# maca/crdt-graph

Measured on AMD Instinct MI355X. Metric: merged ops/sec (whole node) on 10M-op batch, higher is better.
Workload: dtype int64; 1 GPU; flat10m: 10000000 ops per GPU, one document per GPU; replicas=64, window=256, guard=0, parallelism=documents sharded by id over 1 GPU(s)

## Files before the change

crdt-graph_amd/csrc/merge.hip:

```cpp

#include <cstring>

#include "engine.h"
#include "listrank.h"
#include "scan.h"

namespace crdtm {


struct Work {
  uint8_t* st;
  uint32_t* cur;
  uint32_t* leaf;
  uint32_t* addpar;
  uint32_t* dtime;
  uint8_t* dead;
  uint32_t* maxadd;
  uint4* nrec;
  uint32_t* tag;
};

__device__ __forceinline__ uint32_t op_len(const OpsDev& o, uint32_t i) { return o.off[i + 1] - o.off[i]; }

struct Quad {
  uint32_t cnt;
  uint8_t kind[4];
  long long ts[4];
  uint32_t off[5];
};

__device__ __forceinline__ void load_quad(const OpsDev& o, uint32_t i0, Quad& q) {
  if (i0 + 4 <= o.n) {
    q.cnt = 4;
    const uchar4 k = *reinterpret_cast<const uchar4*>(o.kind + i0);
    q.kind[0] = k.x;
    q.kind[1] = k.y;
    q.kind[2] = k.z;
    q.kind[3] = k.w;
    const longlong2 a = *reinterpret_cast<const longlong2*>(o.ts + i0);
    const longlong2 b = *reinterpret_cast<const longlong2*>(o.ts + i0 + 2);
    q.ts[0] = a.x;
    q.ts[1] = a.y;
    q.ts[2] = b.x;
    q.ts[3] = b.y;
    const uint4 f = *reinterpret_cast<const uint4*>(o.off + i0);
    q.off[0] = f.x;
    q.off[1] = f.y;
    q.off[2] = f.z;
    q.off[3] = f.w;
    q.off[4] = o.off[i0 + 4];
  } else {
    q.cnt = o.n - i0;
#pragma unroll
    for (uint32_t k = 0; k < 4; ++k) {
      const bool v = k < q.cnt;
      q.kind[k] = v ? o.kind[i0 + k] : 0;
      q.ts[k] = v ? o.ts[i0 + k] : 0;
    }
#pragma unroll
    for (uint32_t k = 0; k < 5; ++k) q.off[k] = k <= q.cnt ? o.off[i0 + k] : 0;
  }
}

__device__ __forceinline__ void store_quad_u8(uint8_t* p, uint32_t i0, uint32_t cnt, const uint8_t v[4]) {
  if (cnt == 4) {
    *reinterpret_cast<uchar4*>(p + i0) = make_uchar4(v[0], v[1], v[2], v[3]);
  } else {
    for (uint32_t k = 0; k < cnt; ++k) p[i0 + k] = v[k];
  }
}

#define QUAD_LOOP(i0, n)                                                                           \
  for (uint32_t i0 = 4 * (blockIdx.x * blockDim.x + threadIdx.x); i0 < (n); i0 += 4 * gridDim.x * blockDim.x)

#define QUAD_LOOP_XCD(i0, n)                                                                       \
  const uint32_t nq_ = ((n) + 3) / 4;                                                              \
  const bool x8_ = (gridDim.x & 7) == 0;                                                           \
  const uint32_t xc_ = x8_ ? blockIdx.x & 7 : 0, xy_ = x8_ ? blockIdx.x >> 3 : blockIdx.x;         \
  const uint32_t cq_ = (x8_ ? gridDim.x >> 3 : gridDim.x) * blockDim.x, xs_ = x8_ ? 8 : 1;         \
  for (uint32_t j_ = xc_, qd_ = xc_ * cq_ + xy_ * blockDim.x + threadIdx.x, i0 = 4 * qd_;         \
       j_ * cq_ < nq_; j_ += xs_, qd_ = j_ * cq_ + xy_ * blockDim.x + threadIdx.x, i0 = 4 * qd_)   \
    if (qd_ < nq_)

static uint32_t env_grid(const char* name, uint32_t def) {
  const char* e = getenv(name);
  const int g = e ? atoi(e) : 0;
  return g >= 8 && g <= (1 << 20) ? static_cast<uint32_t>(g) : def;
}

inline uint32_t quad_grid(uint64_t n) {
  const uint64_t g = (((n + 3) / 4) + BLOCK - 1) / BLOCK;
  if (g >= 2048) return 2048;
  return g < 8 ? static_cast<uint32_t>(g ? g : 1) : static_cast<uint32_t>((g + 7) & ~7ULL);
}



constexpr uint32_t REP_DIRECT = 4096;
constexpr uint32_t PRE_T = 1024;
template <uint32_t PB>
__global__ void __launch_bounds__(PB) __attribute__((amdgpu_waves_per_eu(PB == 1024 ? 8 : 4, 8))) k_pre(OpsDev o, uint2* rng, DevResult* dres) {
  __shared__ __attribute__((aligned(16))) uint32_t rlo[REP_DIRECT];
  __shared__ __attribute__((aligned(16))) uint32_t rhi[REP_DIRECT];
  for (uint32_t j = threadIdx.x; j < REP_DIRECT / 4; j += blockDim.x) {
    reinterpret_cast<uint4*>(rlo)[j] = make_uint4(NONE, NONE, NONE, NONE);
    reinterpret_cast<uint4*>(rhi)[j] = make_uint4(0u, 0u, 0u, 0u);
  }
  __syncthreads();
  uint32_t mx = 0, bad = 0, neg = 0, ndel = 0, maxr = 0;
  auto fold = [&](const Quad& q) {
#pragma unroll
    for (uint32_t k = 0; k < 4; ++k) {
      if (k >= q.cnt) break;
      const uint32_t L = q.off[k + 1] - q.off[k];
      mx = max(mx, L);
      if (q.kind[k] != CRDTM_ADD) {
        ++ndel;
        continue;
      }
      const long long ts = q.ts[k];
      if (ts >= TWO53 || ts <= -TWO53) {
        bad = 1;
      } else if (ts < 0) {
        neg = 1;
      } else if (L >= 1 && ts != 0) {
        const uint32_t r = static_cast<uint32_t>(static_cast<uint64_t>(ts) >> 32), c = static_cast<uint32_t>(ts);
        maxr = max(maxr, r);
        if (r < REP_DIRECT) {
          if (c < rlo[r]) atomicMin(&rlo[r], c);
          if (c > rhi[r]) atomicMax(&rhi[r], c);
        } else {
          atomicMin(&rng[r].x, c);
          atomicMax(&rng[r].y, c);
        }
      }
    }
  };
  {
    const uint32_t qs = 4 * gridDim.x * blockDim.x;
    uint32_t i0 = 4 * (blockIdx.x * blockDim.x + threadIdx.x);
    for (; i0 + qs < o.n; i0 += 2 * qs) {
      Quad qa, qb;
      load_quad(o, i0, qa);
      load_quad(o, i0 + qs, qb);
      fold(qa);
      fold(qb);
    }
    if (i0 < o.n) {
      Quad qa;
      load_quad(o, i0, qa);
      fold(qa);
    }
  }
  auto mxf = [](uint32_t a, uint32_t b) { return a > b ? a : b; };
  maxr = block_reduce_t<PB>(maxr, 0u, mxf);
  for (uint32_t j = threadIdx.x; j <= maxr && j < REP_DIRECT; j += blockDim.x) {
    if (rlo[j] <= rhi[j]) {
      atomicMin(&rng[j].x, rlo[j]);
      atomicMax(&rng[j].y, rhi[j]);
    }
  }
  mx = block_reduce_t<PB>(mx, 0u, mxf);
  bad = block_reduce_t<PB>(bad, 0u, mxf);
  neg = block_reduce_t<PB>(neg, 0u, mxf);
  ndel = block_reduce_t<PB>(ndel, 0u, [](uint32_t a, uint32_t b) { return a + b; });
  if (threadIdx.x == 0) {
    if (mx) atomicMax(&dres->max_len, mx);
    if (bad) atomicOr(&dres->bad_range, 1u);
    if (neg) atomicOr(&dres->has_negative, 1u);
    if (ndel) atomicAdd(&dres->n_del, ndel);
    if (maxr) atomicMax(&dres->max_replica, maxr);
  }
}

__global__ void __launch_bounds__(BLOCK) k_path_range(OpsDev o, DevResult* dres) {
  const uint64_t np = o.n_path, npair = np / 2;
  auto out = [](long long v) { return v >= TWO53 || v <= -TWO53; };
  uint32_t bad = 0;
  const uint64_t ps = static_cast<uint64_t>(gridDim.x) * blockDim.x;
  uint64_t p = blockIdx.x * static_cast<uint64_t>(blockDim.x) + threadIdx.x;
  for (; p + 3 * ps < npair; p += 4 * ps) {
    longlong2 v[4];
#pragma unroll
    for (uint32_t u = 0; u < 4; ++u) v[u] = *reinterpret_cast<const longlong2*>(o.path + 2 * (p + u * ps));
#pragma unroll
    for (uint32_t u = 0; u < 4; ++u)
      if (out(v[u].x) || out(v[u].y)) bad = 1;
  }
  for (; p < npair; p += ps) {
    const longlong2 v = *reinterpret_cast<const longlong2*>(o.path + 2 * p);
    if (out(v.x) || out(v.y)) bad = 1;
  }
  if ((np & 1) && blockIdx.x == 0 && threadIdx.x == 0 && out(o.path[np - 1])) bad = 1;
  bad = block_max(bad);
  if (threadIdx.x == 0 && bad) atomicOr(&dres->bad_range, 1u);
}

constexpr uint32_t REP_SPEC = 256;
template <uint32_t PB, bool BLIND>
__global__ void __launch_bounds__(PB) k_pre_ts(const long long* __restrict__ ts, const uint8_t* __restrict__ kind,
                                               const uint32_t* __restrict__ off, uint32_t n, uint2* rng,
                                               uint32_t* base, DevResult* dres) {
  __shared__ uint32_t rlo[REP_SPEC], rhi[REP_SPEC];
  __shared__ uint32_t s_last;
  __shared__ unsigned long long sw[PB / 64];
  for (uint32_t j = threadIdx.x; j < REP_SPEC; j += PB) {
    rlo[j] = NONE;
    rhi[j] = 0;
  }
  __syncthreads();
  uint32_t bad = 0, neg = 0, maxr = 0, vfail = 0;
  auto fold = [&](long long t) {
    if (t >= TWO53 || t <= -TWO53) {
      bad = 1;
    } else if (t < 0) {
      neg = 1;
    } else if (t != 0) {
      const uint32_t r = static_cast<uint32_t>(static_cast<uint64_t>(t) >> 32), c = static_cast<uint32_t>(t);
      maxr = max(maxr, r);
      if (r < REP_SPEC) {
        if (BLIND || c < rlo[r]) atomicMin(&rlo[r], c);
        if (BLIND || c > rhi[r]) atomicMax(&rhi[r], c);
      }
    }
  };
  {
    const longlong2* t2 = reinterpret_cast<const longlong2*>(ts);
    const uchar2* k2 = reinterpret_cast<const uchar2*>(kind);
    const uint2* o2 = reinterpret_cast<const uint2*>(off);
    auto verify = [&](uint32_t p, uchar2 k, uint2 f) {
      vfail |= (k.x | k.y) != CRDTM_ADD || f.x != 2 * p || f.y != 2 * p + 1;
    };
    const uint32_t np = n / 2, gs = gridDim.x * PB;
    uint32_t p = blockIdx.x * PB + threadIdx.x;
    for (; p + 3 * gs < np; p += 4 * gs) {
      longlong2 v[4];
      uchar2 k[4];
      uint2 f[4];
#pragma unroll
      for (uint32_t u = 0; u < 4; ++u) {
        v[u] = t2[p + u * gs];
        k[u] = k2[p + u * gs];
        f[u] = o2[p + u * gs];
      }
#pragma unroll
      for (uint32_t u = 0; u < 4; ++u) {
        fold(v[u].x);
        fold(v[u].y);
        verify(p + u * gs, k[u], f[u]);
      }
    }
    for (; p < np; p += gs) {
      const longlong2 v = t2[p];
      fold(v.x);
      fold(v.y);
      verify(p, k2[p], o2[p]);
    }
    if (blockIdx.x == 0 && threadIdx.x == 0) {
      if (n & 1) {
        fold(ts[n - 1]);
        vfail |= kind[n - 1] != CRDTM_ADD || off[n - 1] != n - 1;
      }
      vfail |= off[n] != n;
    }
  }
  auto mxf = [](uint32_t a, uint32_t b) { return a > b ? a : b; };
  maxr = block_reduce_t<PB>(maxr, 0u, mxf);
  for (uint32_t j = threadIdx.x; j <= maxr && j < REP_SPEC; j += PB)
    if (rlo[j] <= rhi[j]) {
      atomicMin(&rng[j].x, rlo[j]);
      atomicMax(&rng[j].y, rhi[j]);
    }
  bad = block_reduce_t<PB>(bad, 0u, mxf);
  neg = block_reduce_t<PB>(neg, 0u, mxf);
  vfail = block_reduce_t<PB>(vfail, 0u, mxf);
  if (threadIdx.x == 0) {
    if (vfail) atomicOr(&dres->spec_fail, 1u);
    if (bad) atomicOr(&dres->bad_range, 1u);
    if (neg) atomicOr(&dres->has_negative, 1u);
    if (maxr) atomicMax(&dres->max_replica, maxr);
    s_last = __hip_atomic_fetch_add(&dres->pre_done, 1u, __ATOMIC_ACQ_REL, __HIP_MEMORY_SCOPE_AGENT) ==
             gridDim.x - 1;
  }
  __syncthreads();
  if (!s_last) return;
  const uint32_t nr =
      min(__hip_atomic_load(&dres->max_replica, __ATOMIC_ACQUIRE, __HIP_MEMORY_SCOPE_AGENT), REP_SPEC - 1) + 1;
  const uint32_t lane = threadIdx.x & 63, wave = threadIdx.x / 64;
  unsigned long long sz = 0;
  if (threadIdx.x < nr) {
    const uint32_t lo = __hip_atomic_load(&rng[threadIdx.x].x, __ATOMIC_RELAXED, __HIP_MEMORY_SCOPE_AGENT);
    const uint32_t hi = __hip_atomic_load(&rng[threadIdx.x].y, __ATOMIC_RELAXED, __HIP_MEMORY_SCOPE_AGENT);
    sz = lo <= hi ? static_cast<unsigned long long>(hi - lo) + 1ULL : 0ULL;
  }
  const unsigned long long inc = wave_incl_scan64(sz);
  if (lane == 63) sw[wave] = inc;
  __syncthreads();
  unsigned long long pre = inc - sz, tot = 0;
  for (uint32_t w = 0; w < PB / 64; ++w) {
    if (w < wave) pre += sw[w];
    tot += sw[w];
  }
  if (threadIdx.x < nr) base[threadIdx.x] = static_cast<uint32_t>(pre < NONE ? pre : NONE);
  if (threadIdx.x == 0) {
    const uint32_t q = static_cast<uint32_t>(tot < NONE - 64 ? tot : NONE - 64);
    dres->range_total = q;
    dres->fl_nw = (q + 63) / 64;
  }
}

__global__ void __launch_bounds__(BLOCK) k_work_init(OpsDev o, Work w) {
  GRID_STRIDE(i, o.n) {
    w.st[i] = op_len(o, i) == 0 ? ST_INVALID : ST_PENDING;
    w.cur[i] = o.n;
    w.addpar[i] = NONE;
    w.dtime[i] = NONE;
    w.tag[i] = NONE;
  }
}

__global__ void __launch_bounds__(BLOCK) k_nrec_init(OpsDev o, Work w) {
  GRID_STRIDE(i, o.n) {
    const uint32_t b = o.off[i], L = o.off[i + 1] - b;
    w.nrec[i] = make_uint4(b, L | (static_cast<uint32_t>(ST_PENDING) << 16), NONE, NONE);
  }
}
__device__ __forceinline__ uint32_t nrec_len(const uint4& r) { return r.y & 0xFFFFu; }
__device__ __forceinline__ uint32_t nrec_st(const uint4& r) { return (r.y >> 16) & 0xFFu; }
__device__ __forceinline__ bool nrec_dead(const uint4& r) { return (r.y >> 24) & 1u; }

__global__ void __launch_bounds__(BLOCK) k_range_base(const uint2* rng, uint32_t* base, DevResult* dres) {
  __shared__ unsigned long long sw[BLOCK / 64];
  const uint32_t nr = dres->max_replica + 1;
  const int lane = threadIdx.x & 63, wave = threadIdx.x >> 6;
  unsigned long long carry = 0;
  for (uint32_t r0 = 0; r0 < nr; r0 += BLOCK) {
    const uint32_t r = r0 + threadIdx.x;
    unsigned long long sz = 0;
    if (r < nr) {
      const uint2 g = rng[r];
      sz = g.x <= g.y ? static_cast<unsigned long long>(g.y - g.x) + 1ULL : 0ULL;
    }
    const unsigned long long inc = wave_incl_scan64(sz);
    if (lane == 63) sw[wave] = inc;
    __syncthreads();
    unsigned long long pre = carry + (inc - sz), tot = 0;
    for (int w = 0; w < BLOCK / 64; ++w) {
      if (w < wave) pre += sw[w];
      tot += sw[w];
    }
    if (r < nr) base[r] = static_cast<uint32_t>(pre < NONE ? pre : NONE);
    carry += tot;
    __syncthreads();
  }
  if (threadIdx.x == 0) dres->range_total = static_cast<uint32_t>(carry < NONE ? carry : NONE);
}

__global__ void __launch_bounds__(BLOCK) k_range_reset(uint2* rng, uint32_t nr, const DevResult* dres) {
  if (nr == 0) nr = dres->max_replica + 1;
  GRID_STRIDE(r, nr) rng[r] = make_uint2(NONE, 0u);
}

void range_reset(crdtm_ctx* c, uint32_t nr) {
// ... 2144 lines not shown
struct RunSizeGen {
  static constexpr bool kStriped = true;
  static constexpr bool kEpilogue = false;
  const uint32_t* tk;
  const uint32_t* offk;
  __device__ __forceinline__ bool aligned(uint64_t b) const {
    return ((reinterpret_cast<uintptr_t>(tk + b) | reinterpret_cast<uintptr_t>(offk + b)) & 15) == 0;
  }
  __device__ __forceinline__ uint4 load4(uint64_t b) const {
    const uint4 t = *reinterpret_cast<const uint4*>(tk + b), f = *reinterpret_cast<const uint4*>(offk + b);
    return make_uint4(t.x | (f.x & SEGF), t.y | (f.y & SEGF), t.z | (f.z & SEGF), t.w | (f.w & SEGF));
  }
  __device__ __forceinline__ void load(uint64_t b, uint64_t n, uint32_t* v) const {
#pragma unroll
    for (int j = 0; j < DS_ITEMS; ++j) v[j] = b + j < n ? (tk[b + j] | (offk[b + j] & SEGF)) : 0u;
  }
};

__global__ void __launch_bounds__(BLOCK) k_run_w2(RunArr a, uint32_t Q, const uint32_t* sarr, const uint32_t* pk,
                                                  const uint32_t* xs, const uint32_t* offk) {
  if (a.qd) Q = min(*a.qd, Q);
  RUN_LOOP(k) {
    const uint32_t f = offk[k], r = sarr[k], p = pk[k];
    if (p > Q) continue;
    const uint32_t ex = (f & SEGF) ? 0u : (xs[k - 1] & ~SEGF);
    a.rr[r].y = ex + (f & ~SEGF);
  }
}

__device__ __forceinline__ uint32_t run_S(const uint32_t* xs, uint32_t k) { return k ? xs[k - 1] : 0u; }

__global__ void __launch_bounds__(BLOCK) k_run_gstart(RunArr a, uint32_t Q, const uint32_t* pk, RunMask rm,
                                                      uint32_t* groot) {
  if (a.qd) Q = min(*a.qd, Q);
  const uint32_t R = *a.nR;
  const uint32_t lane = threadIdx.x & 63;
  for (uint32_t k0 = blockIdx.x * blockDim.x; k0 < R; k0 += gridDim.x * blockDim.x) {
    const uint32_t k = k0 + threadIdx.x;
    const uint32_t p = k < R ? pk[k] : Q + 1;
    const uint32_t P = p < Q ? run_of(rm, p) : NONE;
    uint32_t Pp = __shfl_up(P, 1, 64), Pn = __shfl_down(P, 1, 64);
    if (k >= R) continue;
    if (p == Q && (k == 0 || pk[k - 1] != Q)) *groot = k;
    if (p >= Q) continue;
    if (lane == 0) Pp = k ? (pk[k - 1] < Q ? run_of(rm, pk[k - 1]) : NONE) : NONE;
    if (lane == 63 || k + 1 == R) Pn = k + 1 < R && pk[k + 1] < Q ? run_of(rm, pk[k + 1]) : NONE;
    if (Pp != P) a.rr[P].z = k;
    if (Pn != P) a.rr[P].w = k + 1;
  }
}

__global__ void __launch_bounds__(BLOCK) k_run_w(RunArr a, uint32_t Q, const uint32_t* sarr, const uint32_t* pk,
                                                 const uint32_t* xs, const uint32_t* groot, RunMask rm) {
  if (a.qd) Q = min(*a.qd, Q);
  RUN_LOOP(k) {
    const uint32_t r = sarr[k], p = pk[k];
    if (p > Q) continue;
    if (p == Q) {
      a.rr[r].y = run_S(xs, k) - run_S(xs, *groot);
    } else {
      const uint32_t P = run_of(rm, p);
      a.rr[r].y = run_S(xs, k) - run_S(xs, a.rr[P].z) + (p - a.hh[P].x) + 1u;
    }
  }
}

__global__ void __launch_bounds__(BLOCK) k_run_pos(RunArr a, DevResult* dres) {
  RUN_LOOP(r) {
    const uint4 e = a.rr[r];
    uint32_t s = e.y, d = 0;
    for (uint32_t x = e.x; x != NONE;) {
      if (++d > RUN_MAXD) {
        atomicOr(&dres->run_fail, 1u);
        break;
      }
      const uint4 f = a.rr[x];
      s += f.y;
      x = f.x;
    }
    a.posh[r] = s;
  }
}

__global__ void __launch_bounds__(BLOCK) k_run_expand(RunArr a, uint32_t Q, uint32_t K, RunMask rm,
                                                      const uint32_t* pk, const uint32_t* xs, const uint32_t* qc,
                                                      uint32_t* doc, FlatRec fr, uint32_t lds_iters, uint32_t seg) {
  extern __shared__ uint32_t smw[];
  Q = fr.q(Q);
  const uint32_t iters = (Q + gridDim.x * blockDim.x - 1) / (gridDim.x * blockDim.x);
  const bool mlds = iters <= lds_iters;
  const uint32_t wpb = blockDim.x >> 6;
  if (mlds) {
    const uint32_t nw = (Q + 63) >> 6;
    for (uint32_t j = threadIdx.x; j < iters * wpb; j += blockDim.x) {
      const uint32_t w = (blockIdx.x + (j / wpb) * gridDim.x) * wpb + j % wpb;
      const unsigned long long m = w < nw ? rm.hm[w] : 0ULL;
      smw[3 * j] = static_cast<uint32_t>(m);
      smw[3 * j + 1] = static_cast<uint32_t>(m >> 32);
      smw[3 * j + 2] = w < nw ? rm.hb[w] : 0u;
    }
  }
  __syncthreads();
  const uint32_t lane = threadIdx.x & 63, stride = gridDim.x * blockDim.x;
  const unsigned long long below = (2ULL << lane) - 1ULL;
  auto run_at = [&](uint32_t it, uint32_t q) -> uint32_t {
    unsigned long long mq;
    uint32_t bq;
    if (mlds) {
      const uint32_t* e = smw + 3 * (it * wpb + (threadIdx.x >> 6));
      mq = (static_cast<unsigned long long>(e[1]) << 32) | e[0];
      bq = e[2];
    } else {
      mq = rm.hm[q >> 6];
      bq = rm.hb[q >> 6];
    }
    return bq + static_cast<uint32_t>(__popcll(mq & below)) - 1u;
  };
  uint32_t q0 = blockIdx.x * blockDim.x;
  uint2 hn = make_uint2(0u, ABSENT);
  uint32_t pn = 0;
  uint4 en = make_uint4(0u, 0u, 0u, 0u);
  auto fetch = [&](uint32_t it, uint32_t q) {
    if (q < Q) {
      const uint32_t r = run_at(it, q);
      hn = a.hh[r];
      pn = a.posh[r];
      en = a.rr[r];
    }
  };
  fetch(0, q0 + threadIdx.x);
  for (uint32_t it = 0; q0 < Q; q0 += stride, ++it) {
    const uint32_t q = q0 + threadIdx.x;
    const uint2 h = hn;
    const uint32_t ph = pn;
    const uint4 er = en;
    hn = make_uint2(0u, ABSENT);
    if (q0 + stride < Q) fetch(it + 1, q + stride);
    if (q >= Q || h.y == ABSENT) continue;
    uint32_t p = ph + (q - h.x);
    const uint32_t e0 = er.z, e1 = er.w;
    if (e1 > e0) {
      uint32_t lo = e0, hi = e1;
      while (lo < hi) {
        const uint32_t mid = (lo + hi) >> 1;
        if (pk[mid] < q) lo = mid + 1;
        else hi = mid;
      }
      if (lo > e0) p += seg ? (xs[lo - 1] & ~SEGF) : xs[lo - 1] - run_S(xs, e0);
    }
    if (p < K) doc[p] = 1 + (qc ? qc[q] : q);
  }
}

__global__ void __launch_bounds__(BLOCK) k_fl_count(uint32_t Q, const uint32_t* ep, uint32_t* cnt) {
  uint32_t hot = 0;
  GRID_STRIDE(x, Q) {
    const uint32_t d = ep[x];
    if (d == ABSENT) continue;
    if (d == Q) ++hot;
    else atomicAdd(&cnt[d], 1u);
  }
  hot = block_sum(hot);
  if (threadIdx.x == 0 && hot) atomicAdd(&cnt[Q], hot);
}

thread_local crdtm_ctx* g_prof = nullptr;

void mark_begin(crdtm_ctx* c, hipStream_t st) {
  if (!c->profile) return;
  if (c->pending) hipEventDestroy(c->pending);
  c->pending = nullptr;
  hipEvent_t e;
  if (hipEventCreate(&e) != hipSuccess) return;
  hipEventRecord(e, st);
  c->pending = e;
}

void mark(crdtm_ctx* c, const char* name, hipStream_t st) {
  if (!c->profile || !c->pending) return;
  hipEvent_t e;
  if (hipEventCreate(&e) != hipSuccess) return;
  hipEventRecord(e, st);
  c->marks.push_back({name, c->pending, e});
  c->pending = nullptr;
}

template <class T>
static int grow_array(T*& p, uint64_t old_n, uint64_t new_n) {
  T* q = nullptr;
  HIP_CHECK(hipMalloc(&q, new_n * sizeof(T) + 256));
  if (p) {
    if (old_n) HIP_CHECK(hipMemcpy(q, p, old_n * sizeof(T), hipMemcpyDeviceToDevice));
    HIP_CHECK(hipFree(p));
  }
  p = q;
  return CRDTM_OK;
}

DevStore::~DevStore() {
  void* ps[] = {d.s_key, d.s_next, d.s_src, d.s_child, d.s_dict, d.s_flags, d.d_sent,
                d.d_owner, d.l_kind, d.l_ts, d.l_val, d.l_off, d.l_path, d.doc};
  for (void* p : ps)
    if (p) hipFree(p);
}

static int grow_tree_arrays(crdtm_tree* t, const TreeCaps& need);

int grow_tree(crdtm_tree* t, const TreeCaps& need) {
  if (!t->store) t->store = std::make_shared<DevStore>();
  const int r = grow_tree_arrays(t, need);
  t->store->d = t->d;
  return r;
}

static int grow_tree_arrays(crdtm_tree* t, const TreeCaps& need) {
  HIP_CHECK(hipStreamSynchronize(t->ctx->stream));
  TreeCaps& c = t->cap;
  auto bump = [](uint64_t have, uint64_t want) { return want <= have ? have : (want + want / 4 + 1024); };
  if (need.slots > c.slots) {
    uint64_t n = bump(c.slots, need.slots);
    int r = 0;
    if ((r = grow_array(t->d.s_key, t->n_slots, n)) || (r = grow_array(t->d.s_next, t->n_slots, n)) ||
        (r = grow_array(t->d.s_src, t->n_slots, n)) || (r = grow_array(t->d.s_child, t->n_slots, n)) ||
        (r = grow_array(t->d.s_dict, t->n_slots, n)) || (r = grow_array(t->d.s_flags, t->n_slots, n)))
      return r;
    c.slots = n;
  }
  if (need.dicts > c.dicts) {
    uint64_t n = bump(c.dicts, need.dicts);
    int r = 0;
    if ((r = grow_array(t->d.d_sent, t->n_dicts, n)) || (r = grow_array(t->d.d_owner, t->n_dicts, n))) return r;
    c.dicts = n;
  }
// ... 310 lines not shown
      if ((r = scan_excl_u32(logidx, logidx, n, &dr->log_n, ws, s))) return r;
      if ((r = scan_excl_u32(plen, plen, n, &dr->log_npath, ws, s))) return r;
      LAUNCH(k_log, dim3(g), dim3(BLOCK), 0, s, o, st, t->d, 0u, 0u, logidx, plen);
      LAUNCH(k_log_tail, dim3(1), dim3(1), 0, s, t->d, 0u, &dr->log_n, 0u, &dr->log_npath);
    }
    uint32_t* qc = nullptr;
    if (!fr.qd && Q != K) {
      qc = fb.qc = ws.alloc<uint32_t>(Q);
      LAUNCH(k_fl_present, dim3(gq), dim3(BLOCK), 0, s, Q, fr, qc);
      if ((r = scan_excl_u32(qc, qc, Q, nullptr, ws, s))) return r;
    }
    static const uint32_t mask_u = [] {
      const char* e = getenv("CRDTM_MASK_U");
      const uint32_t u = e ? static_cast<uint32_t>(atoi(e)) : RM_MASK_UNROLL;
      return (u == 1 || u == 4) ? u : RM_MASK_UNROLL;
    }();
    static const uint32_t mask_grid = env_grid("CRDTM_MASK_GRID", 1024);
    const uint32_t gw = std::max<uint32_t>(1, std::min<uint32_t>(mask_grid, (NW + mask_u * (BLOCK / 64) - 1) /
                                                                                 (mask_u * (BLOCK / 64))));
    const size_t mshm = maxr + 1 <= HOST_RANGES ? 3 * (maxr + 1) * sizeof(uint32_t) : 0;
    const bool dq = fr.qd != nullptr;
    auto mask_launch = [&](auto kern, const char* name) {
      prof_begin(s);
      hipLaunchKernelGGL(kern, dim3(gw), dim3(BLOCK), mshm, s, fr, Q, hm, hc, t->d, qc, logidx, o, ix, maxr + 1,
                         check ? dr : nullptr, c->rtab);
      prof_mark(name, s);
    };
    static const bool diag_mask2 = [] {
      const char* e = getenv("CRDTM_DIAG_MASK2");
      return e && e[0] == '1';
    }();
    if (diag_mask2) mask_launch(dq ? k_run_mask<RM_MASK_UNROLL, true> : k_run_mask<RM_MASK_UNROLL, false>, "k_run_mask");
    if (mask_u == 1) mask_launch(dq ? k_run_mask<1, true> : k_run_mask<1, false>, "k_run_mask");
    else if (mask_u == 4) mask_launch(dq ? k_run_mask<4, true> : k_run_mask<4, false>, "k_run_mask");
    else mask_launch(dq ? k_run_mask<RM_MASK_UNROLL, true> : k_run_mask<RM_MASK_UNROLL, false>, "k_run_mask");
    if ((r = dscan<SumOp, false>(ArrGen{hc}, hb, NW, &dr->run_count, ws, s, nullptr, fr.qd ? &dr->fl_nw : nullptr,
                                 "k_dscan_runs")))
      return r;
    static const bool run_v2 = [] {
      const char* e = getenv("CRDTM_RUN_V2");
      return !(e && e[0] == '0');
    }();
    ra.hasch = run_v2 ? ws.alloc<uint8_t>(Q + 1) : nullptr;
    static const uint32_t heads_grid = env_grid("CRDTM_HEADS_GRID", 4096);
    LAUNCH(k_run_heads, dim3(grid_for(64ULL * NW, BLOCK, heads_grid)), dim3(BLOCK), 0, s, fr, Q, fb.rm, ra.hh,
           ra.hasch);
    ra.rr = ws.alloc<uint4>(Q + 1);
    ra.ca = ws.alloc<unsigned long long>(Q + 1);
    uint32_t* kinv = ws.alloc<uint32_t>(Q + 1);
    ra.kinv = kinv;
    ra.posh = ws.alloc<uint32_t>(Q + 1);
    uint32_t* sk[2] = {ws.alloc<uint32_t>(Q + 1), ws.alloc<uint32_t>(Q + 1)};
    uint32_t* sv[2] = {ws.alloc<uint32_t>(Q + 1), ws.alloc<uint32_t>(Q + 1)};
    uint32_t* xs = ws.alloc<uint32_t>(Q + 1);
    uint32_t* groot = fb.cnt;
    static const uint32_t run_grid = env_grid("CRDTM_RUN_GRID", 2048);
    const uint32_t gr = grid_for(Q, BLOCK, run_grid);
    static const bool ep_coh = [] {
      const char* e = getenv("CRDTM_EP_COHERENT");
      return e && e[0] == '1';
    }();
    if (ep_coh) LAUNCH(k_run_ep<true>, dim3(gr), dim3(BLOCK), 0, s, ra, Q, fb.rm, fr, sk[0], sv[0]);
    else LAUNCH(k_run_ep<false>, dim3(gr), dim3(BLOCK), 0, s, ra, Q, fb.rm, fr, sk[0], sv[0]);
    uint32_t *pk = nullptr, *sarr = nullptr;
    {
      uint32_t sbits = 8;
      while (sbits < 32 && ((static_cast<uint64_t>(Q) + 1) >> sbits) != 0) sbits += 8;
      if ((r = radix_sort_pairs(sk[0], sv[0], sk[1], sv[1], ra.nR, Q, sbits, ws, s, &pk, &sarr, kinv))) return r;
      ra.tk = pk == sk[0] ? sk[1] : sk[0];
      if (!run_v2) LAUNCH(k_run_gstart, dim3(gr), dim3(BLOCK), 0, s, ra, Q, pk, fb.rm, groot);
    }
    if (run_v2) {
      uint32_t* offk = ws.alloc<uint32_t>(Q + 1);
      LAUNCH(k_run_sizes, dim3(gr), dim3(BLOCK), 0, s, ra, Q, sarr, pk, fb.rm, offk);
      if ((r = dscan<SegSumOp, true>(RunSizeGen{ra.tk, offk}, xs, Q, nullptr, ws, s, nullptr, ra.nR, "k_dscan_seg")))
        return r;
      LAUNCH(k_run_w2, dim3(gr), dim3(BLOCK), 0, s, ra, Q, sarr, pk, xs, offk);
    } else {
      LAUNCH(k_run_tree_up, dim3(gr), dim3(BLOCK), 0, s, ra, sarr);
      if ((r = dscan<SumOp, true>(ArrGen{ra.tk}, xs, Q, nullptr, ws, s, nullptr, ra.nR, "k_dscan_xs"))) return r;
      LAUNCH(k_run_w, dim3(gr), dim3(BLOCK), 0, s, ra, Q, sarr, pk, xs, groot, fb.rm);
    }
    LAUNCH(k_run_pos, dim3(gr), dim3(BLOCK), 0, s, ra, dr);
    static const uint32_t ex_grid = env_grid("CRDTM_EX_GRID", 2048);
    const uint32_t gx = grid_for(Q, BLOCK, ex_grid);
    const uint32_t ex_iters = (Q + gx * BLOCK - 1) / (gx * BLOCK);
    LAUNCH(k_run_expand, dim3(gx), dim3(BLOCK),
           ex_iters <= EX_ITERS ? 3 * ex_iters * (BLOCK / 64) * sizeof(uint32_t) : 0, s, ra, Q, K, fb.rm, pk, xs, qc,
           t->d.doc, fr, ex_iters <= EX_ITERS ? ex_iters : 0u, run_v2 ? 1u : 0u);
    static const uint32_t next_grid = env_grid("CRDTM_NEXT_GRID", 1u << 20);
    fb.rep = ws.alloc<long long>(2 * static_cast<uint64_t>(maxr) + 2);
    RepCollect rc{o, 0u, c->rtab, fb.rep, &dr->n_replica_out, dr->rep_inline, check ? c->crange : nullptr};
    const bool rep_here = !(all_applied && !log_done);
    if (rep_here) rc.nr = maxr + 1;
    LAUNCH(k_fl_next, dim3(grid_for(K, BLOCK, next_grid)), dim3(BLOCK), 0, s, K, t->d.doc, t->d, t->cap.slots, rc);
    if (rep_here) return CRDTM_OK;
    if (all_applied && !log_done) fl_log_copy(c, o, t->d, simple);
  } else if (all_applied && !log_done) {
    fl_log_copy(c, o, t->d, simple);
  }
  if (!fb.rep) fb.rep = ws.alloc<long long>(2 * static_cast<uint64_t>(maxr) + 2);
  LAUNCH(k_fl_rep_collect, dim3(grid_for(maxr + 1)), dim3(BLOCK), 0, s, o, maxr + 1, c->rtab, fb.rep,
         &dr->n_replica_out, dr->rep_inline, check ? c->crange : nullptr);
  return CRDTM_OK;
}

static int flat_order_fallback(crdtm_tree* t, uint32_t Q, uint32_t K, FlatBufs& fb) {
  crdtm_ctx* c = t->ctx;
  hipStream_t s = c->stream;
  Arena& ws = c->ws;
  DevResult* dr = c->dres;
  const uint32_t U = Q + 1;
  const uint32_t gq = grid_for(Q);
  uint32_t* anc = fb.anc;
  uint32_t* cnt = fb.cnt;
  uint32_t* fill = fb.fill;
  uint32_t* qc = fb.qc;
  int r;
  {
    RunArr ra{};
    ra.hh = fb.hh;
    LAUNCH(k_run_ep_slots, dim3(gq), dim3(BLOCK), 0, s, ra, Q, fb.rm, fb.fr, anc);
  }
  uint32_t* carr = ws.alloc<uint32_t>(U);
  uint32_t* ns = ws.alloc<uint32_t>(U);
  HIP_CHECK(hipMemsetAsync(cnt, 0, (U + 1) * sizeof(uint32_t), s));
  HIP_CHECK(hipMemsetAsync(fill, 0, (U + 1) * sizeof(uint32_t), s));
  LAUNCH(k_fl_count, dim3(grid_for(Q, BLOCK, 2048)), dim3(BLOCK), 0, s, Q, anc, cnt);
  uint32_t* n_child = &dr->n_sentinels;
  if ((r = scan_excl_u32(cnt, cnt, U + 1, n_child, ws, s))) return r;
  LAUNCH(k_fl_scatter, dim3(gq), dim3(BLOCK), 0, s, Q, anc, cnt, fill, carr);
  {
    const uint32_t gb = grid_for(Q, BLOCK, 2048);
    uint32_t* bc = ws.alloc<uint32_t>(gb + 1);
    LAUNCH(k_fl_root_count, dim3(gb), dim3(BLOCK), 0, s, Q, anc, bc);
    if ((r = scan_excl_u32(bc, bc, gb, nullptr, ws, s))) return r;
    LAUNCH(k_fl_root_place, dim3(gb), dim3(BLOCK), 0, s, Q, anc, bc, cnt, carr);
  }
  if ((r = segmented_sort_desc_id(cnt, U, carr, U, ws, s, dr, Q))) return r;
  LAUNCH(k_fl_links, dim3(gq), dim3(BLOCK), 0, s, anc, cnt, n_child, carr, ns);
  if ((r = list_rank_fused(FlatEulerSrc{Q, anc, cnt, carr, ns}, 2ULL * U, 2 * Q, FlatDocSink{Q, t->d.doc, qc},
                           ws, s)))
    return r;
  LAUNCH(k_fl_next, dim3(grid_for(K)), dim3(BLOCK), 0, s, K, t->d.doc, t->d, t->cap.slots, RepCollect{});
  return CRDTM_OK;
}

static int apply_flat(crdtm_tree* t, const OpsDev& o, const TsIndex& ix, uint32_t Q, uint32_t maxr, uint8_t* st,
                      uint8_t* st_out, crdtm_result* res, bool simple, RangeReset& rr, bool devq = false,
                      bool* done = nullptr) {
  if (done) *done = true;
  crdtm_ctx* c = t->ctx;
  hipStream_t s = c->stream;
  Arena& ws = c->ws;
  DevResult* dr = c->dres;
  const uint32_t n = o.n;
  const uint32_t g = grid_for(n);
  const uint32_t U = Q + 1;
  FlatBufs fb{};
  fb.anc = ws.alloc<uint32_t>(U);
  fb.cnt = ws.alloc<uint32_t>(U + 1);
  fb.fill = ws.alloc<uint32_t>(U + 1);
  int r;
  auto grow_for = [&](uint32_t K, uint32_t applied) -> int {
    TreeCaps need = t->cap;
    need.slots = std::max<uint64_t>(need.slots, 1ULL + K + 1);
    need.dicts = std::max<uint64_t>(need.dicts, 2);
    need.log = std::max<uint64_t>(need.log, t->log_n + applied + 1);
    need.lpath = std::max<uint64_t>(need.lpath, t->log_npath + o.n_path + 1);
    need.doc = std::max<uint64_t>(need.doc, 1ULL + K);
    if (need.slots > t->cap.slots || need.dicts > t->cap.dicts || need.log > t->cap.log ||
        need.lpath > t->cap.lpath || need.doc > t->cap.doc)
      return grow_tree(t, need);
// ... 75 lines not shown
    LAUNCH(k_reset_root, dim3(1), dim3(1), 0, s, t->d.s_next, nullptr);
    launch_pre(c, o, s);
    LAUNCH(k_range_base, dim3(1), dim3(BLOCK), 0, s, c->crange, const_cast<uint32_t*>(ix.base), dr);
    rr.armed = true;
  }
  LAUNCH(k_fl_rep_collect, dim3(grid_for(maxr + 1)), dim3(BLOCK), 0, s, o, maxr + 1, c->rtab, nullptr, nullptr,
         nullptr, nullptr);
  LAUNCH(k_fl_stat_reset, dim3(1), dim3(1), 0, s, dr);
  LAUNCH(k_fl_status, dim3(quad_grid(n)), dim3(BLOCK), 0, s, o, st, ix, Q, fb.fr, t->timestamp, c->rtab, dr);
  if ((r = sync_read(c))) return r;
  if (c->hres->dup_fix) {
    LAUNCH(k_fl_rep_collect, dim3(grid_for(maxr + 1)), dim3(BLOCK), 0, s, o, maxr + 1, c->rtab, nullptr, nullptr,
           nullptr, nullptr);
    LAUNCH(k_fl_stat_reset, dim3(1), dim3(1), 0, s, dr);
    LAUNCH(k_fl_status, dim3(quad_grid(n)), dim3(BLOCK), 0, s, o, st, ix, Q, fb.fr, t->timestamp, c->rtab, dr);
    if ((r = sync_read(c))) return r;
  }
  const DevResult h1 = *c->hres;
  if (h1.bad_range) return CRDTM_E_RANGE;
  uint32_t guard = 0;
  const long long new_ts = t->timestamp + h1.own_ok_adds - t->own_bias;
  if (replica_of(new_ts) != replica_of(t->timestamp)) guard |= G_REPLICA_DRIFT;
  res->guard = guard;
  if (guard || h1.err_index != NONE)
    LAUNCH(k_fl_rep_collect, dim3(grid_for(maxr + 1)), dim3(BLOCK), 0, s, o, maxr + 1, c->rtab, nullptr, nullptr,
           nullptr, nullptr);
  if (guard) {
    r = run_replay(t, o, st, res, guard);
    if (r == CRDTM_OK && st_out)
      LAUNCH(k_status_out, dim3(g), dim3(BLOCK), 0, s, st, n,
             res->err_index >= 0 ? static_cast<uint32_t>(res->err_index) : NONE, st_out);
    return r;
  }
  res->path_taken = CRDTM_PATH_CLOSED_FORM;
  if (h1.err_index != NONE) {
    uint8_t est = 0;
    HIP_CHECK(hipMemcpy(&est, st + h1.err_index, 1, hipMemcpyDeviceToHost));
    res->code = est == ST_INVALID ? CRDTM_INVALID_PATH : CRDTM_OPERATION_FAILED;
    res->err_index = h1.err_index;
    if (st_out) LAUNCH(k_status_out, dim3(g), dim3(BLOCK), 0, s, st, n, h1.err_index, st_out);
    return CRDTM_OK;
  }
  const uint32_t K = h1.n_adds_applied;
  const bool all_applied = h1.n_applied == n;
  if ((r = grow_for(K, h1.n_applied))) return r;
  LAUNCH(k_fl_commit_reset, dim3(1), dim3(1), 0, s, dr);
  if ((r = flat_order_commit(t, o, ix, Q, maxr, st, K, all_applied, spec, simple, false, fb))) return r;
  if (st_out) LAUNCH(k_status_out, dim3(g), dim3(BLOCK), 0, s, st, n, NONE, st_out);
  if ((r = sync_read(c))) return r;
  if (c->hres->run_fail && (r = flat_order_fallback(t, Q, K, fb))) return r;
  return finish(K, h1.n_applied, h1.n_already, all_applied ? o.n_path : c->hres->log_npath, new_ts);
}

static int apply_core(crdtm_tree* t, const OpsDev& o, uint8_t* st_out, crdtm_result* res) {
  crdtm_ctx* c = t->ctx;
  hipStream_t s = c->stream;
  Arena& ws = c->ws;
  const uint32_t n = o.n;
  res->err_index = -1;
  res->code = CRDTM_OK;
  if (n == 0) {
    res->path_taken = CRDTM_PATH_CLOSED_FORM;
    t->last_begin = t->last_end = t->log_n;
    return CRDTM_OK;
  }
  Work w;
  w.st = ws.alloc<uint8_t>(n);
  uint32_t* rbase = ws.alloc<uint32_t>(RID_SLOTS + 1);
  DevResult* dr = c->dres;
  const bool dres_ready = c->dres_ready;
  c->dres_ready = false;
  const char* fe = getenv("CRDTM_FORCE_REPLAY");
  const bool force_replay = fe && fe[0] == '1';
  static const bool spec_on = [] {
    const char* e = getenv("CRDTM_FLAT_SPEC");
    return !(e && e[0] == '0');
  }();
  if (spec_on && !force_replay && t->n_slots == 1 && t->log_n == 0 && !t->remerge && o.n_path == n) {
    uint32_t b = 8;
    while (b < 32 && ((static_cast<uint64_t>(n) + 2) >> b) != 0) b += 8;
    const uint64_t qcap = std::min<uint64_t>(std::max<uint64_t>((1ULL << b) - 2, 65536), 4ULL * n + 65536);
    if (qcap + 2 < (1ULL << FR_ABITS) - 1) {
      if (!dres_ready) LAUNCH(k_dres_init, dim3(1), dim3(64), 0, s, dr);
      static const uint32_t pre_grid = env_grid("CRDTM_PRE_GRID", 256);
      static const bool pre_blind = [] {
        const char* e = getenv("CRDTM_PRE_BLIND");
        return e && e[0] == '1';
      }();
      const uint32_t gp = static_cast<uint32_t>(std::min<uint64_t>((n / 2 + PRE_T - 1) / PRE_T + 1, pre_grid));
      if (pre_blind)
        LAUNCH((k_pre_ts<PRE_T, true>), dim3(gp), dim3(PRE_T), 0, s, o.ts, o.kind, o.off, n, c->crange, rbase, dr);
      else
        LAUNCH((k_pre_ts<PRE_T, false>), dim3(gp), dim3(PRE_T), 0, s, o.ts, o.kind, o.off, n, c->crange, rbase, dr);
      RangeReset spec_clean{c};
      TsIndex ix;
      ix.rng = c->crange;
      ix.base = rbase;
      ix.dense = 1;
      ix.h = TsHash{nullptr, nullptr, 0};
      ix.first = nullptr;
      bool done = false;
      int rs = apply_flat(t, o, ix, static_cast<uint32_t>(qcap), REP_SPEC - 1, w.st, st_out, res, true, spec_clean,
                          true, &done);
      if (rs || done) return rs;
    }
  }
  LAUNCH(k_dres_init, dim3(1), dim3(64), 0, s, dr);
  launch_pre(c, o, s);
  LAUNCH(k_range_base, dim3(1), dim3(BLOCK), 0, s, c->crange, rbase, dr);
  RangeReset keep_clean{c};
  int r;
  if ((r = sync_read(c))) return r;
  keep_clean.nr = c->hres->max_replica + 1;
  if (c->hres->bad_range) return CRDTM_E_RANGE;
  const uint32_t maxlen = c->hres->max_len;
  if (t->max_depth < maxlen) t->max_depth = maxlen;
  const uint32_t g = grid_for(n);
  if (force_replay || t->n_slots != 1 || t->log_n != 0) {
    if (o.n_path) {
      LAUNCH(k_path_range, dim3(std::min<uint32_t>(grid_for(o.n_path / 2 + 1), 1024)), dim3(BLOCK), 0, s, o, dr);
      if ((r = sync_read(c))) return r;
      if (c->hres->bad_range) return CRDTM_E_RANGE;
    }
    r = run_replay(t, o, w.st, res, force_replay ? G_FORCED : G_NOT_FRESH);
    if (r == CRDTM_OK && st_out)
      LAUNCH(k_status_out, dim3(g), dim3(BLOCK), 0, s, w.st, n,
             res->err_index >= 0 ? static_cast<uint32_t>(res->err_index) : NONE, st_out);
    return r;
  }
  const uint32_t maxr = c->hres->max_replica;
  const uint64_t range_total = c->hres->range_total;
  TsIndex ix;
  ix.rng = c->crange;
  ix.base = rbase;
  ix.dense = (!c->hres->has_negative && range_total <= 4ULL * n + 65536) ? 1u : 0u;
  const bool flat = maxlen == 1 && c->hres->n_del == 0;
  const bool levels = !flat && maxlen <= MAXLV_BUCKET;
  const bool side_range = !(ix.dense && flat) && !levels && o.n_path;
  if (side_range) {
    HIP_CHECK(hipEventRecord(c->ev_fork, s));
    HIP_CHECK(hipStreamWaitEvent(c->side, c->ev_fork, 0));
    LAUNCH(k_path_range, dim3(std::min<uint32_t>(grid_for(o.n_path / 2 + 1), 1024)), dim3(BLOCK), 0, c->side, o,
           dr);
    HIP_CHECK(hipEventRecord(c->ev_join, c->side));
  }
  auto range_ok = [&]() -> int {
    return c->hres->bad_range ? CRDTM_E_RANGE : CRDTM_OK;
  };
  if (ix.dense) {
    ix.h = TsHash{nullptr, nullptr, 0};
    ix.first = nullptr;
    if (flat)
      return apply_flat(t, o, ix, static_cast<uint32_t>(range_total), maxr, w.st, st_out, res, o.n_path == n,
                        keep_clean);
    ix.first = ws.alloc<uint32_t>(range_total + 1);
    HIP_CHECK(hipMemsetAsync(ix.first, 0xFF, (range_total + 1) * sizeof(uint32_t), s));
    const uint32_t nrep = maxr + 1 <= HOST_RANGES ? maxr + 1 : 0u;
    LAUNCH(k_index_store, dim3(quad_grid(n)), dim3(BLOCK), 3 * nrep * sizeof(uint32_t), s, o, ix, nrep);
    LAUNCH(k_index_fix, dim3(quad_grid(n)), dim3(BLOCK), 3 * nrep * sizeof(uint32_t), s, o, ix, nrep);
  } else {
    const uint32_t H = pow2_at_least(2 * static_cast<uint64_t>(n));
    ix.first = nullptr;
    ix.h.keys = ws.alloc<unsigned long long>(H);
    ix.h.vals = ws.alloc<uint32_t>(H);
    ix.h.mask = H - 1;
    HIP_CHECK(hipMemsetAsync(ix.h.keys, 0, H * sizeof(unsigned long long), s));
    HIP_CHECK(hipMemsetAsync(ix.h.vals, 0xFF, H * sizeof(uint32_t), s));
// ... 585 lines not shown
```

Before: 16.67 billion ops/s.

## Software-pipeline pre-pass loads, batch run_expand searches, skip redundant global atomics

The timestamp pre-pass now double-buffers groups of four loads so the next group is in flight while the current one is folded, with a masked tail loop. The run_expand kernel is templated on the LDS mode and processes two queries per thread, interleaving their binary searches so memory loads overlap. Global atomicMin, atomicMax and max_replica updates are skipped when a relaxed load shows they would not change the value. Grid env lookups are re-read under test hooks, and the extra live registers may reduce occupancy.

```diff
diff --git a/crdt-graph_amd/csrc/merge.hip b/crdt-graph_amd/csrc/merge.hip
--- a/crdt-graph_amd/csrc/merge.hip
+++ b/crdt-graph_amd/csrc/merge.hip
@@ -87,6 +87,11 @@
   const int g = e ? atoi(e) : 0;
   return g >= 8 && g <= (1 << 20) ? static_cast<uint32_t>(g) : def;
 }
+#define TUNED_GRID(name, def)                           \
+  ([] {                                                 \
+    static const uint32_t g_ = env_grid(name, def);     \
+    return test_hooks() ? env_grid(name, def) : g_;     \
+  }())
 
 inline uint32_t quad_grid(uint64_t n) {
   const uint64_t g = (((n + 3) / 4) + BLOCK - 1) / BLOCK;
@@ -232,29 +237,68 @@
       vfail |= (k.x | k.y) != CRDTM_ADD || f.x != 2 * p || f.y != 2 * p + 1;
     };
     const uint32_t np = n / 2, gs = gridDim.x * PB;
-    uint32_t p = blockIdx.x * PB + threadIdx.x;
-    for (; p + 3 * gs < np; p += 4 * gs) {
+    struct Grp {
       longlong2 v[4];
       uchar2 k[4];
       uint2 f[4];
+    };
+    auto load = [&](Grp& g, uint32_t p) {
 #pragma unroll
       for (uint32_t u = 0; u < 4; ++u) {
-        v[u] = t2[p + u * gs];
-        k[u] = k2[p + u * gs];
-        f[u] = o2[p + u * gs];
-      }
+        g.v[u] = t2[p + u * gs];
+        g.k[u] = k2[p + u * gs];
+        g.f[u] = o2[p + u * gs];
+      }
+    };
+    auto eat = [&](const Grp& g, uint32_t p) {
 #pragma unroll
       for (uint32_t u = 0; u < 4; ++u) {
+        fold(g.v[u].x);
+        fold(g.v[u].y);
+        verify(p + u * gs, g.k[u], g.f[u]);
+      }
+    };
+    const uint32_t G = 4 * gs;
+    uint32_t p = blockIdx.x * PB + threadIdx.x;
+    const uint32_t pl = blockIdx.x * PB + (PB - 1) + 3 * gs;
+    if (pl < np) {
+      uint32_t left = (np - 1 - pl) / G;
+      Grp a, b;
+      load(a, p);
+      for (; left >= 2; left -= 2, p += 2 * G) {
+        load(b, p + G);
+        eat(a, p);
+        load(a, p + 2 * G);
+        eat(b, p + G);
+      }
+      if (left) {
+        load(b, p + G);
+        eat(a, p);
+        eat(b, p + G);
+        p += 2 * G;
+      } else {
+        eat(a, p);
+        p += G;
+      }
+    }
+    for (; p < np; p += G) {
+      longlong2 v[4];
+      uchar2 k[4];
+      uint2 f[4];
+#pragma unroll
+      for (uint32_t u = 0; u < 4; ++u) {
+        const uint32_t pu = p + u * gs < np ? p + u * gs : p;
+        v[u] = t2[pu];
+        k[u] = k2[pu];
+        f[u] = o2[pu];
+      }
+#pragma unroll
+      for (uint32_t u = 0; u < 4; ++u) {
+        if (p + u * gs >= np) break;
         fold(v[u].x);
         fold(v[u].y);
         verify(p + u * gs, k[u], f[u]);
       }
-    }
-    for (; p < np; p += gs) {
-      const longlong2 v = t2[p];
-      fold(v.x);
-      fold(v.y);
-      verify(p, k2[p], o2[p]);
     }
     if (blockIdx.x == 0 && threadIdx.x == 0) {
       if (n & 1) {
@@ -268,8 +312,10 @@
   maxr = block_reduce_t<PB>(maxr, 0u, mxf);
   for (uint32_t j = threadIdx.x; j <= maxr && j < REP_SPEC; j += PB)
     if (rlo[j] <= rhi[j]) {
-      atomicMin(&rng[j].x, rlo[j]);
-      atomicMax(&rng[j].y, rhi[j]);
+      const uint32_t glo = __hip_atomic_load(&rng[j].x, __ATOMIC_RELAXED, __HIP_MEMORY_SCOPE_AGENT);
+      const uint32_t ghi = __hip_atomic_load(&rng[j].y, __ATOMIC_RELAXED, __HIP_MEMORY_SCOPE_AGENT);
+      if (rlo[j] < glo) atomicMin(&rng[j].x, rlo[j]);
+      if (rhi[j] > ghi) atomicMax(&rng[j].y, rhi[j]);
     }
   bad = block_reduce_t<PB>(bad, 0u, mxf);
   neg = block_reduce_t<PB>(neg, 0u, mxf);
@@ -278,7 +324,8 @@
     if (vfail) atomicOr(&dres->spec_fail, 1u);
     if (bad) atomicOr(&dres->bad_range, 1u);
     if (neg) atomicOr(&dres->has_negative, 1u);
-    if (maxr) atomicMax(&dres->max_replica, maxr);
+    if (maxr > __hip_atomic_load(&dres->max_replica, __ATOMIC_RELAXED, __HIP_MEMORY_SCOPE_AGENT))
+      atomicMax(&dres->max_replica, maxr);
     s_last = __hip_atomic_fetch_add(&dres->pre_done, 1u, __ATOMIC_ACQ_REL, __HIP_MEMORY_SCOPE_AGENT) ==
              gridDim.x - 1;
   }
@@ -2589,13 +2636,14 @@
   }
 }
 
+template <bool MLDS>
 __global__ void __launch_bounds__(BLOCK) k_run_expand(RunArr a, uint32_t Q, uint32_t K, RunMask rm,
                                                       const uint32_t* pk, const uint32_t* xs, const uint32_t* qc,
-                                                      uint32_t* doc, FlatRec fr, uint32_t lds_iters, uint32_t seg) {
+                                                      uint32_t* doc, FlatRec fr, uint32_t seg) {
   extern __shared__ uint32_t smw[];
   Q = fr.q(Q);
   const uint32_t iters = (Q + gridDim.x * blockDim.x - 1) / (gridDim.x * blockDim.x);
-  const bool mlds = iters <= lds_iters;
+  constexpr bool mlds = MLDS;
   const uint32_t wpb = blockDim.x >> 6;
   if (mlds) {
     const uint32_t nw = (Q + 63) >> 6;
@@ -2611,51 +2659,84 @@
   const uint32_t lane = threadIdx.x & 63, stride = gridDim.x * blockDim.x;
   const unsigned long long below = (2ULL << lane) - 1ULL;
   auto run_at = [&](uint32_t it, uint32_t q) -> uint32_t {
+    const bool ok = q < Q;
     unsigned long long mq;
     uint32_t bq;
     if (mlds) {
-      const uint32_t* e = smw + 3 * (it * wpb + (threadIdx.x >> 6));
+      const uint32_t* e = smw + 3 * ((ok ? it : 0u) * wpb + (threadIdx.x >> 6));
       mq = (static_cast<unsigned long long>(e[1]) << 32) | e[0];
       bq = e[2];
     } else {
-      mq = rm.hm[q >> 6];
-      bq = rm.hb[q >> 6];
-    }
-    return bq + static_cast<uint32_t>(__popcll(mq & below)) - 1u;
+      const uint32_t w = ok ? q >> 6 : 0u;
+      mq = rm.hm[w];
+      bq = rm.hb[w];
+    }
+    return ok ? bq + static_cast<uint32_t>(__popcll(mq & below)) - 1u : 0u;
   };
+  constexpr uint32_t W = 2;
   uint32_t q0 = blockIdx.x * blockDim.x;
-  uint2 hn = make_uint2(0u, ABSENT);
-  uint32_t pn = 0;
-  uint4 en = make_uint4(0u, 0u, 0u, 0u);
+  uint2 hn[W];
+  uint32_t pn[W];
+  uint4 en[W];
   auto fetch = [&](uint32_t it, uint32_t q) {
-    if (q < Q) {
-      const uint32_t r = run_at(it, q);
-      hn = a.hh[r];
-      pn = a.posh[r];
-      en = a.rr[r];
+    uint32_t r[W];
+#pragma unroll
+    for (uint32_t u = 0; u < W; ++u) r[u] = run_at(it + u, q + u * stride);
+#pragma unroll
+    for (uint32_t u = 0; u < W; ++u) {
+      hn[u] = a.hh[r[u]];
+      pn[u] = a.posh[r[u]];
+      en[u] = a.rr[r[u]];
     }
   };
+  if (Q == 0) return;
   fetch(0, q0 + threadIdx.x);
-  for (uint32_t it = 0; q0 < Q; q0 += stride, ++it) {
-    const uint32_t q = q0 + threadIdx.x;
-    const uint2 h = hn;
-    const uint32_t ph = pn;
-    const uint4 er = en;
-    hn = make_uint2(0u, ABSENT);
-    if (q0 + stride < Q) fetch(it + 1, q + stride);
-    if (q >= Q || h.y == ABSENT) continue;
-    uint32_t p = ph + (q - h.x);
-    const uint32_t e0 = er.z, e1 = er.w;
-    if (e1 > e0) {
-      uint32_t lo = e0, hi = e1;
-      while (lo < hi) {
-        const uint32_t mid = (lo + hi) >> 1;
-        if (pk[mid] < q) lo = mid + 1;
-        else hi = mid;
-      }
-      if (lo > e0) p += seg ? (xs[lo - 1] & ~SEGF) : xs[lo - 1] - run_S(xs, e0);
-    }
-    if (p < K) doc[p] = 1 + (qc ? qc[q] : q);
+  for (uint32_t it = 0; q0 < Q; q0 += W * stride, it += W) {
+    uint32_t q[W], p[W], e0[W], lo[W], hi[W];
+    bool on[W];
+#pragma unroll
+    for (uint32_t u = 0; u < W; ++u) {
+      q[u] = q0 + threadIdx.x + u * stride;
+      on[u] = q[u] < Q && hn[u].y != ABSENT;
+      p[u] = pn[u] + (q[u] - hn[u].x);
+      e0[u] = en[u].z;
+      lo[u] = e0[u];
+      hi[u] = on[u] && en[u].w > e0[u] ? en[u].w : e0[u];
+    }
+    fetch(it + W, q[0] + W * stride);
+    bool any = false;
+#pragma unroll
+    for (uint32_t u = 0; u < W; ++u) any |= lo[u] < hi[u];
+    while (any) {
+      uint32_t mid[W], v[W];
+#pragma unroll
+      for (uint32_t u = 0; u < W; ++u) {
+        mid[u] = (lo[u] + hi[u]) >> 1;
+        v[u] = pk[lo[u] < hi[u] ? mid[u] : 0u];
+      }
+      any = false;
+#pragma unroll
+      for (uint32_t u = 0; u < W; ++u) {
+        if (lo[u] < hi[u]) {
+          if (v[u] < q[u]) lo[u] = mid[u] + 1;
+          else hi[u] = mid[u];
+        }
+        any |= lo[u] < hi[u];
+      }
+    }
+    uint32_t x1[W], x0[W];
+#pragma unroll
+    for (uint32_t u = 0; u < W; ++u) {
+      const bool add = on[u] && lo[u] > e0[u];
+      x1[u] = xs[add ? lo[u] - 1 : 0u];
+      if (!add) x1[u] = 0u;
+      x0[u] = add && !seg ? run_S(xs, e0[u]) : 0u;
+    }
+#pragma unroll
+    for (uint32_t u = 0; u < W; ++u) {
+      p[u] += seg ? (x1[u] & ~SEGF) : x1[u] - x0[u];
+      if (on[u] && p[u] < K) doc[p[u]] = 1 + (qc ? qc[q[u]] : q[u]);
+    }
   }
 }
 
@@ -3132,13 +3213,16 @@
       LAUNCH(k_run_w, dim3(gr), dim3(BLOCK), 0, s, ra, Q, sarr, pk, xs, groot, fb.rm);
     }
     LAUNCH(k_run_pos, dim3(gr), dim3(BLOCK), 0, s, ra, dr);
-    static const uint32_t ex_grid = env_grid("CRDTM_EX_GRID", 2048);
+    const uint32_t ex_grid = TUNED_GRID("CRDTM_EX_GRID", 2048);
     const uint32_t gx = grid_for(Q, BLOCK, ex_grid);
     const uint32_t ex_iters = (Q + gx * BLOCK - 1) / (gx * BLOCK);
-    LAUNCH(k_run_expand, dim3(gx), dim3(BLOCK),
-           ex_iters <= EX_ITERS ? 3 * ex_iters * (BLOCK / 64) * sizeof(uint32_t) : 0, s, ra, Q, K, fb.rm, pk, xs, qc,
-           t->d.doc, fr, ex_iters <= EX_ITERS ? ex_iters : 0u, run_v2 ? 1u : 0u);
-    static const uint32_t next_grid = env_grid("CRDTM_NEXT_GRID", 1u << 20);
+    if (ex_iters <= EX_ITERS)
+      LAUNCH(k_run_expand<true>, dim3(gx), dim3(BLOCK), 3 * ex_iters * (BLOCK / 64) * sizeof(uint32_t), s, ra, Q, K,
+             fb.rm, pk, xs, qc, t->d.doc, fr, run_v2 ? 1u : 0u);
+    else
+      LAUNCH(k_run_expand<false>, dim3(gx), dim3(BLOCK), 0, s, ra, Q, K, fb.rm, pk, xs, qc, t->d.doc, fr,
+             run_v2 ? 1u : 0u);
+    const uint32_t next_grid = TUNED_GRID("CRDTM_NEXT_GRID", 1u << 20);
     fb.rep = ws.alloc<long long>(2 * static_cast<uint64_t>(maxr) + 2);
     RepCollect rc{o, 0u, c->rtab, fb.rep, &dr->n_replica_out, dr->rep_inline, check ? c->crange : nullptr};
     const bool rep_here = !(all_applied && !log_done);
@@ -3380,7 +3464,7 @@
     const uint64_t qcap = std::min<uint64_t>(std::max<uint64_t>((1ULL << b) - 2, 65536), 4ULL * n + 65536);
     if (qcap + 2 < (1ULL << FR_ABITS) - 1) {
       if (!dres_ready) LAUNCH(k_dres_init, dim3(1), dim3(64), 0, s, dr);
-      static const uint32_t pre_grid = env_grid("CRDTM_PRE_GRID", 256);
+      const uint32_t pre_grid = TUNED_GRID("CRDTM_PRE_GRID", 256);
       static const bool pre_blind = [] {
         const char* e = getenv("CRDTM_PRE_BLIND");
         return e && e[0] == '1';
```

Result: no change. 16.77 billion ops/s (median of 6 runs) (+0.6%).
